# HengyiWang/spann3r

Measured on AMD Instinct MI355X. Metric: frames/sec/GPU (224px, 10-frame seq) + mem-bank cross-attn HBM GB/s, higher is better.
Workload: dtype bf16; 1 GPU; Spann3R.forward, 10-frame 224x224 sequence, batch 1, ViT-L enc / ViT-B dec / DPT heads, eval memory policy; parallelism=sequences sharded 1/GPU x1, hip_graphs=True

## Files before the change

include/spann3r_hip.h:

```cpp
#ifndef SPANN3R_HIP_H
#define SPANN3R_HIP_H

#include <stdint.h>

#ifdef __cplusplus
extern "C" {
#endif

enum { SP3_F32 = 0, SP3_BF16 = 1 };
enum { SP3_ATTN_F32X3 = 2, SP3_ATTN_F16X3 = 3 };
enum { SP3_ACT_NONE = 0, SP3_ACT_GELU = 1, SP3_ACT_RELU = 2 };
enum { SP3_EPI_PLAIN = 0, SP3_EPI_ROPE_VT = 1, SP3_EPI_PIXSHUF = 2, SP3_EPI_PARTIAL = 3 };
enum { SP3_LOAD_PLAIN = 0, SP3_LOAD_CONV3X3 = 1, SP3_LOAD_SOFTMAX = 2 };

const char* sp3_last_error(void);
int sp3_version(void);

int sp3_weight_stream_set(int mode);
int sp3_weight_stream_get(void);

typedef struct sp3_gemm_desc {
  const float* A;
  const float* A2;
  const void* W;
// ... 151 lines not shown
int sp3_gather_cols(const void* src, int64_t ld_src, void* dst, int64_t ld_dst, const int32_t* sel, int n_sel,
                    int n_fill, int C, int elem_size, void* stream);
int sp3_gather_1d(const float* src, float* dst, const int32_t* sel, int n_sel, void* stream);

int sp3_conv3x3_tile(const void* x, int in_bf16, const void* w_packed, const float* bias, const float* res1,
                     const float* res2, void* out, int out_bf16, int res_bf16, int tile_px, int B, int H, int W,
                     int Cin, int Cout, int relu_in, int act, void* stream);
int sp3_im2col_patch(const float* img, int64_t sb, int64_t sc, int64_t sy, int64_t sx, int B, int C, int H, int W,
                     int p, void* out, int out_bf16, int out_packed, void* stream);
int sp3_upsample2x(const float* in, float* out, int B, int H, int W, int C, int outH, int outW, void* stream);
int sp3_upsample2x_bf16(const void* in, void* out, int B, int H, int W, int C, int outH, int outW, void* stream);
int sp3_head_final(const float* feat, const float* w, const float* b, int64_t pixels, int C, float* pts,
                   float* conf, float* raw, void* stream);
int sp3_head_final_bf16(const void* feat, const float* w, const float* b, int64_t pixels, int C, float* pts, float* conf,
                        float* raw, void* stream);

int sp3_preprocess_image(const uint8_t* src, int64_t src_row_stride, int crop_l, int crop_t, int H1, int W1,
                         const int32_t* hbounds, const int32_t* hcoef, int hksize, int W2,
                         const int32_t* vbounds, const int32_t* vcoef, int vksize, int H2,
                         int crop2_l, int crop2_t, int outW, int outH, int transpose, uint8_t* tmp, float* out, void* stream);

int64_t sp3_conf_loss_ws_bytes(int n, int B);
int sp3_conf_loss_forward(const float* P, const float* Cf, const float* G, const uint8_t* V, const float* pose0, int n, int B, int HW,
                          float alpha, int fix_first, void* ws, float* out7, float* ent_out, void* stream);
int sp3_conf_loss_backward(const float* P, const float* Cf, const float* G, const uint8_t* V, const float* pose0, int n, int B, int HW,
                           float alpha, int fix_first, const void* ws, const float* grad_scale2, float* dP, float* dC, void* stream);
int64_t sp3_ssi_loss_ws_bytes(int n, int B, int HW);
int sp3_ssi_loss_forward(const float* P, const float* G, const uint8_t* V, const float* pose0, int n, int B, int HW, int fix_first,
                         int gt_scale, void* ws, float* out, void* stream);
int sp3_ssi_align_stats(const float* P, const float* G, const uint8_t* V, const float* pose0, int n, int B, int HW, void* ws, float* stats,
// ... 353 lines not shown
```

spann3r_amd/csrc/common.h:

```cpp
#pragma once
#include <hip/hip_runtime.h>
#include <stdint.h>
#include <stdio.h>
#include "../../include/spann3r_hip.h"

typedef __attribute__((ext_vector_type(8))) __bf16 bf16x8;
typedef __attribute__((ext_vector_type(4))) __bf16 bf16x4;
typedef __attribute__((ext_vector_type(2))) __bf16 bf16x2;
typedef __attribute__((ext_vector_type(4))) float f32x4;

#define SP3_WAVE 64

void sp3_set_error(const char* fmt, ...);

#define SP3_CHECK(cond, ...)                     \
  do {                                           \
    if (!(cond)) {                               \
      sp3_set_error(__VA_ARGS__);                \
      return 1;                                  \
    }                                            \
  } while (0)

#define SP3_LAUNCH_CHECK(what)                                              \
  do {                                                                      \
// ... 107 lines not shown
  return t;
}
__device__ __forceinline__ float up2x_mix(const Up2xTaps& t, float v00, float v01, float v10, float v11) {
  const float top = __fmaf_rn(t.hx, v00, __fmul_rn(t.lx, v01)), bot = __fmaf_rn(t.hx, v10, __fmul_rn(t.lx, v11));
  return __fmaf_rn(t.hy, top, __fmul_rn(t.ly, bot));
}

__device__ __forceinline__ int64_t packed_off(int row, int k, int K, bool bf16) {
  const int lkb = bf16 ? 6 : 5, lch = bf16 ? 4 : 3;
  const int nkb = (K + (1 << lkb) - 1) >> lkb;
  const int kb = k >> lkb, kk = k & ((1 << lkb) - 1);
  const int g = kk >> lch, e = kk & ((1 << lch) - 1);
  const int h = e >> (lch - 1), eh = e & ((1 << (lch - 1)) - 1);
  return (((((int64_t)(row >> 4) * nkb + kb) * 2 + h) * 4 + g) * 16 + (row & 15)) * (1 << (lch - 1)) + eh;
}
```

spann3r_amd/csrc/conv.hip:

```cpp
#include "common.h"
#include <type_traits>
#include <cstdlib>

namespace {

constexpr int TH = 8, TW = 8;
constexpr int HP = (TH + 2) * (TW + 2);
constexpr int BM = TH * TW, BN = 64;
constexpr int MF = BM / 16, NF = BN / 16;
constexpr int SLAB_LD = BN + 4;
constexpr int DEPTH = 3;
constexpr int SP3_CONV_WIDE_MIN_WGS = 256;

struct ConvArgs {
  const void* x; const __bf16* w; const float* bias; const float* res1; const float* res2; void* out;
  int B, H, W, Cin, Cout, tiles_x, tiles_y, relu_in, act, out_bf16;
  int xcd_nb;
};

__device__ __forceinline__ bool conv_tile_of(const ConvArgs& a, int& t, int& nblk) {
  t = blockIdx.x; nblk = blockIdx.y;
  if (a.xcd_nb) {
    const unsigned L = blockIdx.x, xc = L & 7, jj = L >> 3, q = jj / (unsigned)a.xcd_nb;
    nblk = (int)(jj - q * a.xcd_nb);
// ... 371 lines not shown

template <typename TIN, int NF, bool WS>
int launch(dim3 grid, hipStream_t st, const ConvArgs& a) {
  constexpr int lds = lds_bytes<NF>();
  auto kern = conv3x3_wide_kernel<TIN, NF, 0, WS>;
  if (lds > 64 * 1024) {
    static bool raised = false;
    if (!raised) {
      hipError_t e = hipFuncSetAttribute(reinterpret_cast<const void*>(kern), hipFuncAttributeMaxDynamicSharedMemorySize, lds);
      if (e != hipSuccess) { sp3_set_error("sp3_conv3x3_tile: cannot raise dynamic LDS to %d: %s", lds, hipGetErrorString(e)); return 2; }
      raised = true;
    }
  }
  hipLaunchKernelGGL(kern, grid, dim3(256), lds, st, a);
  return 0;
}
}

}

extern "C" int sp3_conv3x3_tile(const void* x, int in_bf16, const void* w_packed, const float* bias, const float* res1,
                                const float* res2, void* out, int out_bf16, int res_bf16, int tile_px, int B, int H, int W,
                                int Cin, int Cout, int relu_in, int act, void* stream) {
  SP3_CHECK(x && w_packed && out, "sp3_conv3x3_tile: null pointer");
  SP3_CHECK(B > 0 && H > 0 && W > 0, "sp3_conv3x3_tile: bad shape");
  SP3_CHECK(Cin % 64 == 0 && Cin >= 64 && Cout % 64 == 0 && Cout >= 64, "sp3_conv3x3_tile: Cin=%d / Cout=%d must be multiples of 64", Cin, Cout);
  SP3_CHECK(act == SP3_ACT_NONE || act == SP3_ACT_RELU, "sp3_conv3x3_tile: act %d", act);
  SP3_CHECK(out_bf16 == 0 || out_bf16 == 1, "sp3_conv3x3_tile: out_bf16 %d is not 0 or 1", out_bf16);
  SP3_CHECK(res_bf16 == 0 || res_bf16 == 1, "sp3_conv3x3_tile: res_bf16 %d is not 0 or 1", res_bf16);
  SP3_CHECK(tile_px >= 0 && tile_px <= 3, "sp3_conv3x3_tile: tile_px %d is not 0..3", tile_px);
// ... 38 lines not shown
  auto launch = [&](auto kern) -> int {
    static size_t raised = 0;
    if (lds > 64 * 1024 && lds > raised) {
      raised = lds;
      hipError_t e = hipFuncSetAttribute(reinterpret_cast<const void*>(kern), hipFuncAttributeMaxDynamicSharedMemorySize, (int)lds);
      if (e != hipSuccess) { sp3_set_error("sp3_conv3x3_tile: cannot raise dynamic LDS to %zu: %s", lds, hipGetErrorString(e)); return 2; }
    }
    hipLaunchKernelGGL(kern, grid, dim3(256), lds, st, a);
    return 0;
  };
  const int rc = in_bf16 ? launch(conv3x3_tile_kernel<__bf16>) : launch(conv3x3_tile_kernel<float>);
  if (rc) return rc;
  SP3_LAUNCH_CHECK("sp3_conv3x3_tile");
  return 0;
}
```

spann3r_amd/csrc/dpt.hip:

```cpp
#include "common.h"
#include <math.h>

namespace {

__global__ __launch_bounds__(256) void im2col_patch_kernel(const float* __restrict__ img, int64_t sb, int64_t sc, int64_t sy,
                                                           int64_t sx, int C, int H, int W, int p, void* __restrict__ out,
                                                           int out_bf16, int out_packed, int64_t total) {
  const int64_t idx = (int64_t)blockIdx.x * 256 + threadIdx.x;
  if (idx >= total) return;
  const int K = C * p * p;
  const int64_t row = idx / K;
  const int k = (int)(idx - row * K);
  const int nw = W / p, nh = H / p;
  const int b = (int)(row / (nh * nw));
  const int rem = (int)(row - (int64_t)b * nh * nw);
  const int ty = rem / nw, tx = rem - ty * nw;
  const int c = k / (p * p), r2 = k - c * p * p;
  const int iy = r2 / p, ix = r2 - iy * p;
  const float val = img[b * sb + c * sc + (int64_t)(ty * p + iy) * sy + (int64_t)(tx * p + ix) * sx];
  const int64_t o = out_packed ? packed_off((int)row, k, K, out_bf16 != 0) : idx;
  if (out_bf16) reinterpret_cast<__bf16*>(out)[o] = (__bf16)val;
  else reinterpret_cast<float*>(out)[o] = val;
}

// ... 91 lines not shown
    const float4 w1 = *reinterpret_cast<const float4*>(w + C + c);
    const float4 w2 = *reinterpret_cast<const float4*>(w + 2 * C + c);
    const float4 w3 = *reinterpret_cast<const float4*>(w + 3 * C + c);
    a0 += (x.x * w0.x + x.y * w0.y) + (x.z * w0.z + x.w * w0.w);
    a1 += (x.x * w1.x + x.y * w1.y) + (x.z * w1.z + x.w * w1.w);
    a2 += (x.x * w2.x + x.y * w2.y) + (x.z * w2.z + x.w * w2.w);
    a3 += (x.x * w3.x + x.y * w3.y) + (x.z * w3.z + x.w * w3.w);
  }
#pragma unroll
  for (int o = 1; o < 8; o <<= 1) {
    a0 += __shfl_xor(a0, o); a1 += __shfl_xor(a1, o); a2 += __shfl_xor(a2, o); a3 += __shfl_xor(a3, o);
  }
  if (valid && sub == 0) {
    const float x = a0 + bias[0], y = a1 + bias[1], z = a2 + bias[2], c = a3 + bias[3];
    if (raw) { raw[pix * 4 + 0] = x; raw[pix * 4 + 1] = y; raw[pix * 4 + 2] = z; raw[pix * 4 + 3] = c; }
    const float d = sqrtf(x * x + y * y + z * z);
    const float sc = expm1f(d) / fmaxf(d, 1e-8f);
    pts[pix * 3 + 0] = x * sc; pts[pix * 3 + 1] = y * sc; pts[pix * 3 + 2] = z * sc;
    conf[pix] = 1.0f + expf(c);
  }
}

template <int LP, int PPT>
__global__ __launch_bounds__(256) void head_final_bf16x8_kernel(const __bf16* __restrict__ feat, const float* __restrict__ w,
                                                                const float* __restrict__ bias, int64_t pixels, float* __restrict__ pts,
                                                                float* __restrict__ conf, float* __restrict__ raw) {
  constexpr int C = 8 * LP, PPB = 256 / LP;
  const int li = threadIdx.x % LP, pl = threadIdx.x / LP;
  float wr[4][8];
#pragma unroll
  for (int f = 0; f < 4; ++f) {
    const float4 a = *reinterpret_cast<const float4*>(w + f * C + li * 8), b = *reinterpret_cast<const float4*>(w + f * C + li * 8 + 4);
    wr[f][0] = a.x; wr[f][1] = a.y; wr[f][2] = a.z; wr[f][3] = a.w; wr[f][4] = b.x; wr[f][5] = b.y; wr[f][6] = b.z; wr[f][7] = b.w;
  }
// ... 12 lines not shown
    float a[4];
#pragma unroll
    for (int f = 0; f < 4; ++f) {
      float t0 = 0.f, t1 = 0.f;
#pragma unroll
      for (int e = 0; e < 4; ++e) { t0 = fmaf((float)x[q][e], wr[f][e], t0); t1 = fmaf((float)x[q][4 + e], wr[f][4 + e], t1); }
      a[f] = t0 + t1;
    }
#pragma unroll
    for (int o = 1; o < LP; o <<= 1) {
      a[0] += __shfl_xor(a[0], o); a[1] += __shfl_xor(a[1], o); a[2] += __shfl_xor(a[2], o); a[3] += __shfl_xor(a[3], o);
    }
    if (li == 0 && pix < pixels) {
      const float X = a[0] + b0, Y = a[1] + b1, Z = a[2] + b2, Cc = a[3] + b3;
      if (raw) *reinterpret_cast<float4*>(raw + pix * 4) = make_float4(X, Y, Z, Cc);
      const float d = sqrtf(X * X + Y * Y + Z * Z);
      const float sc = expm1f(d) / fmaxf(d, 1e-8f);
      pts[pix * 3 + 0] = X * sc; pts[pix * 3 + 1] = Y * sc; pts[pix * 3 + 2] = Z * sc;
      conf[pix] = 1.0f + expf(Cc);
    }
  }
}

}

#define ST(s) reinterpret_cast<hipStream_t>(s)

extern "C" int sp3_im2col_patch(const float* img, int64_t sb, int64_t sc, int64_t sy, int64_t sx, int B, int C, int H, int W,
                                int p, void* out, int out_bf16, int out_packed, void* stream) {
  SP3_CHECK(img && out && B > 0 && C > 0 && p > 0, "sp3_im2col_patch: bad arguments");
  SP3_CHECK(H % p == 0 && W % p == 0, "Input image size (%d,%d) is not a multiple of patch size (%d)", H, W, p);
  const int64_t total = (int64_t)B * (H / p) * (W / p) * C * p * p;
  hipLaunchKernelGGL(im2col_patch_kernel, dim3((unsigned)((total + 255) / 256)), dim3(256), 0, ST(stream), img, sb, sc, sy, sx,
                     C, H, W, p, out, out_bf16, out_packed, total);
// ... 57 lines not shown
```

spann3r_amd/engine.py:

```python
import math
import os

import torch

from . import ops
from .lib import ACT_NONE, ACT_GELU, ACT_RELU
from .config import Spann3RConfig


def _rope_tables(max_pos, base, device):
    half = 32
    inv_freq = 1.0 / (base ** (torch.arange(0, half, 2).float() / half))
    t = torch.arange(max_pos, dtype=torch.float32)
    ang = torch.einsum("i,j->ij", t, inv_freq)
    return ang.cos().contiguous().to(device), ang.sin().contiguous().to(device)


def _rope_tables_narrow(max_pos, base, head_dim, device):
    D = head_dim // 2
    nf = D // 2
    assert nf <= 16 and head_dim % 4 == 0
    inv_freq = 1.0 / (base ** (torch.arange(0, D, 2).float() / D))
    t = torch.arange(max_pos, dtype=torch.float32)
    ang = torch.einsum("i,j->ij", t, inv_freq)
# ... 576 lines not shown
        if x1 is not None:
            s = self.ws("fus_sum_" + tag, (M, F), self.mdt)
            self._rcu(x1, pre + "u1", B, H, W_, s, extra_res=x0, tag=tag, c1_done=c1_done, extra_up=x0_up)
            cur = s
        r = self.ws("fus_rcu2_" + tag, (M, F), self.mdt)
        self._rcu(cur, pre + "u2", B, H, W_, r, tag=tag, c1_done=c1_done and x1 is None)
        oc = self.ws("fus_oc_" + tag, (M, F), self.mdt)
        ops.gemm(r, w[pre + "out.w"], oc, M=M, N=F, K=F, lda=F, ldc=F, bias=w[pre + "out.b"])
        OH, OW = (2 * H, 2 * W_) if crop is None else crop
        if fold_up:
            return oc, OH, OW
        up = self.ws("fus_up_" + tag, (B * OH * OW, F), self.mdt)
        ops.upsample2x(oc, up, B=B, H=H, W_=W_, C_=F, outH=OH, outW=OW)
        return up, OH, OW

    def dpt_head(self, dec, B, nh, nw, num, want_raw=False):
        self.activate()
        cfg, w = self.cfg, self.w
        F, Lc = cfg.dpt_feat, cfg.dpt_last
        pre = "dpt%d." % num
        R = B * nh * nw
        hk = cfg.hooks
        dims = (cfg.enc_dim, cfg.dec_dim, cfg.dec_dim, cfg.dec_dim)
        ld = (96, 192, 384, 768)
        mdt = self.mdt
        t = [self.ws("dpt%d_pp%d" % (num, i), (R, ld[i]), mdt) for i in range(4)]
        import contextlib
        lv = ops.HEAD_LEVELS
        group = ops.level if len({dec[hk[i]].dtype for i in range(4)}) == 1 else contextlib.nullcontext
        with (group if lv else contextlib.nullcontext)():
            for i0 in (0, 2):
# ... 39 lines not shown
            for i in range(4):
                layer_rn(i)
        path, up, Hc, Wc = rn[3], None, h3, w3
        for j in range(4):
            Hn, Wn = geo[3 - j]
            fold = lv and j < 3 and ops.conv3x3_takes_res2_up(w[refs[j + 1][0] + "u1c2.w"], mdt, B, *geo[2 - j])
            nxt, OH_, OW_ = self._fusion(refs[j][0], B, Hn, Wn, path, rn[3 - j] if j else None, refs[j][1], crop=(nh, nw) if j == 0 else None,
                                         c1_done=lv, x0_up=up, fold_up=fold)
            path, up = nxt, ((Hn, Wn) if fold else None)
        p1, H1, W1 = path, OH_, OW_
        a = self.ws("dpt%d_h0" % num, (B * H1 * W1, Lc), mdt)
        ops.conv3x3(p1, w[pre + "h0.w"], a, B=B, H=H1, W_=W1, Cin=F, Cout=Lc, bias=w[pre + "h0.b"])
        OH, OW = 2 * H1, 2 * W1
        u = self.ws("dpt%d_h0up" % num, (B * OH * OW, Lc), mdt)
        ops.upsample2x(a, u, B=B, H=H1, W_=W1, C_=Lc)
        c = self.ws("dpt%d_h2" % num, (B * OH * OW, Lc), mdt)
        ops.conv3x3(u, w[pre + "h2.w"], c, B=B, H=OH, W_=OW, Cin=Lc, Cout=Lc, bias=w[pre + "h2.b"], act=ACT_RELU)
        pts = self.ws("dpt_pts%d" % num, (B, OH, OW, 3))
        conf = self.ws("dpt_conf%d" % num, (B, OH, OW))
        raw = self.ws("dpt_raw%d" % num, (B, OH, OW, 4)) if want_raw else None
        ops.head_final(c, w[pre + "h4.w"], w[pre + "h4.b"], B * OH * OW, Lc, pts, conf, raw)
        return pts, conf, raw

    def encode_cur_value_feat(self, tok, out, res, pos32=None):
        self.activate()
        cfg, w = self.cfg, self.w
        B, P, Cv = tok.shape
        assert Cv == cfg.val_dim
        R, E = B * P, cfg.enc_dim
        zero_pos = self.ws("valf_zero_pos", (R, 2), torch.int32, zero=True)
        rope_tab = None
        if cfg.mem_pos_enc:
            assert pos32 is not None and self.rope_narrow is not None
            zero_pos, rope_tab = pos32, self.rope_narrow
        x = self.ws("valf_x", (R, Cv))
        xpA, xpB = self.wsp("valf_xpA", R, Cv), self.wsp("valf_xpB", R, Cv)
        stA, stB = self.stats("valf_stA", R, Cv), self.stats("valf_stB", R, Cv)
        ops.copy2d(tok.reshape(R, Cv), Cv, x, Cv, R, Cv)
        ops.pack_stats(x, xpA, stA, rows=R, C_=Cv)
        for i in range(cfg.val_depth):
            self._block(x, xpA, stA, xpB, stB, R, B, P, Cv, cfg.enc_heads, "val%d." % i, zero_pos, tag="_valf",
                        head_dim=Cv // cfg.enc_heads, rope_tab=rope_tab)
        ops.gemm(xpA, w["value_out.w"], out, M=R, N=E, K=Cv, lda=Cv, ldc=E, bias=w["value_out.b"], res1=res, ldr1=E,
                 ln=ops.LnFold(stA, Cv, w["value_out.s"], 1e-6))
        return out

    def encode_cur_value(self, pts3d, out, res):
        self.activate()
        cfg, w = self.cfg, self.w
        B, H, W_, _ = pts3d.shape
        p, E = cfg.patch, cfg.enc_dim
        nh, nw = H // p, W_ // p
        P = nh * nw
        R = B * P
        _, pos32, zero_pos = self.positions(B, nh, nw)
        col = self.wsp("im2col_val", R, 3 * p * p)
        sb, sy, sx, sc = pts3d.stride()
        ops.im2col_patch(pts3d, col, B=B, C_=3, H=H, W_=W_, p=p, strides=(sb, sc, sy, sx))
        x, xp, st = self._vit(col, R, B, P, "pospatch", "val", cfg.val_depth, pos32 if cfg.mem_pos_enc else zero_pos, tag="_val")
        ops.gemm(xp, w["value_out.w"], out, M=R, N=E, K=E, lda=E, ldc=E, bias=w["value_out.b"], res1=res, ldr1=E,
                 ln=ops.LnFold(st, E, w["value_out.s"], 1e-6))
        return out
```

spann3r_amd/lib.py:

```python
import ctypes as C
import os

import torch

_HERE = os.path.dirname(os.path.abspath(__file__))
LIB_PATH = os.environ.get("SP3_LIB_PATH") or os.path.join(_HERE, "libspann3r_hip.so")

F32, BF16 = 0, 1
ATTN_F32X3, ATTN_F16X3 = 2, 3
ACT_NONE, ACT_GELU, ACT_RELU = 0, 1, 2
EPI_PLAIN, EPI_ROPE_VT, EPI_PIXSHUF, EPI_PARTIAL = 0, 1, 2, 3
LOAD_PLAIN, LOAD_CONV3X3, LOAD_SOFTMAX = 0, 1, 2


class GemmDesc(C.Structure):
    _fields_ = [
        ("A", C.c_void_p), ("A2", C.c_void_p), ("W", C.c_void_p), ("C", C.c_void_p), ("bias", C.c_void_p),
        ("res1", C.c_void_p), ("res2", C.c_void_p),
        ("M", C.c_int32), ("N", C.c_int32), ("K", C.c_int32), ("batch", C.c_int32),
        ("K1", C.c_int32),
        ("lda", C.c_int64), ("lda2", C.c_int64), ("ldw", C.c_int64), ("ldc", C.c_int64),
        ("ldr1", C.c_int64), ("ldr2", C.c_int64),
        ("strideA", C.c_int64), ("strideW", C.c_int64), ("strideC", C.c_int64),
        ("alpha", C.c_float), ("wdtype", C.c_int32), ("act", C.c_int32), ("out_bf16", C.c_int32),
# ... 158 lines not shown
    "sp3_cos_sim": [C.c_void_p, C.c_void_p, C.c_int, C.c_int, C.c_int, C.c_void_p, C.c_void_p, C.c_void_p],
    "sp3_mem_append": [C.c_void_p, C.c_void_p, C.c_int, C.c_int, C.c_void_p],
    "sp3_bank_state_set": [C.c_void_p, C.c_int, C.c_int, C.c_void_p],
    "sp3_prob_merge": [C.c_void_p, C.c_void_p, C.c_int, C.c_int, C.c_int, C.c_void_p, C.c_void_p],
    "sp3_colsum_prob": [C.c_void_p, C.c_void_p, C.c_int, C.c_int, C.c_int, C.c_void_p, C.c_void_p, C.c_void_p],
    "sp3_cos_sim_state": [C.c_void_p, C.c_void_p, C.c_int, C.c_int, C.c_int, C.c_void_p, C.c_void_p, C.c_void_p, C.c_void_p],
    "sp3_prune_select": [C.c_void_p, C.c_void_p, C.c_int, C.c_float, C.c_int, C.c_void_p, C.c_void_p],
    "sp3_gather_rows": [C.c_void_p, C.c_void_p, C.c_void_p, C.c_int, C.c_int, C.c_int, C.c_void_p],
    "sp3_gather_cols": [C.c_void_p, C.c_int64, C.c_void_p, C.c_int64, C.c_void_p, C.c_int, C.c_int, C.c_int,
                        C.c_int, C.c_void_p],
    "sp3_gather_1d": [C.c_void_p, C.c_void_p, C.c_void_p, C.c_int, C.c_void_p],
    "sp3_im2col_patch": [C.c_void_p, C.c_int64, C.c_int64, C.c_int64, C.c_int64, C.c_int, C.c_int, C.c_int, C.c_int,
                         C.c_int, C.c_void_p, C.c_int, C.c_int, C.c_void_p],
    "sp3_conv3x3_tile": [C.c_void_p, C.c_int, C.c_void_p, C.c_void_p, C.c_void_p, C.c_void_p, C.c_void_p, C.c_int, C.c_int, C.c_int,
                         C.c_int, C.c_int, C.c_int, C.c_int, C.c_int, C.c_int, C.c_int, C.c_void_p],
    "sp3_upsample2x": [C.c_void_p, C.c_void_p, C.c_int, C.c_int, C.c_int, C.c_int, C.c_int, C.c_int, C.c_void_p],
    "sp3_head_final": [C.c_void_p, C.c_void_p, C.c_void_p, C.c_int64, C.c_int, C.c_void_p, C.c_void_p, C.c_void_p,
                       C.c_void_p],
    "sp3_upsample2x_bf16": [C.c_void_p, C.c_void_p, C.c_int, C.c_int, C.c_int, C.c_int, C.c_int, C.c_int, C.c_void_p],
    "sp3_head_final_bf16": [C.c_void_p, C.c_void_p, C.c_void_p, C.c_int64, C.c_int, C.c_void_p, C.c_void_p, C.c_void_p,
                            C.c_void_p],
    "sp3_fill_f32": [C.c_void_p, C.c_float, C.c_int64, C.c_void_p],
    "sp3_cast_f32_to_bf16": [C.c_void_p, C.c_void_p, C.c_int64, C.c_void_p],
    "sp3_copy2d_f32": [C.c_void_p, C.c_int64, C.c_void_p, C.c_int64, C.c_int, C.c_int, C.c_void_p],
    "sp3_spin": [C.c_int64, C.c_void_p, C.c_void_p],
    "sp3_conf_loss_forward": [C.c_void_p, C.c_void_p, C.c_void_p, C.c_void_p, C.c_void_p, C.c_int, C.c_int, C.c_int, C.c_float, C.c_int,
                              C.c_void_p, C.c_void_p, C.c_void_p, C.c_void_p],
    "sp3_conf_loss_backward": [C.c_void_p, C.c_void_p, C.c_void_p, C.c_void_p, C.c_void_p, C.c_int, C.c_int, C.c_int, C.c_float, C.c_int,
                               C.c_void_p, C.c_void_p, C.c_void_p, C.c_void_p, C.c_void_p],
    "sp3_transpose": [C.c_void_p, C.c_int64, C.c_void_p, C.c_int64, C.c_int, C.c_int, C.c_void_p],
# ... 231 lines not shown
```

spann3r_amd/model.py:

```python
import argparse
import collections
import os
import weakref

import torch
import torch.nn as nn

from . import ops
from .config import Spann3RConfig, FULL
from .engine import Engine
from .weights import param_spec, alias_of, synth_state_dict


def _build_param_tree(root: nn.Module, spec):
    made = {}
    for key, shape in spec.items():
        parts = key.split(".")
        mod = root
        for name in parts[:-1]:
            if not hasattr(mod, name) or not isinstance(getattr(mod, name), nn.Module):
                mod.add_module(name, nn.Module())
            mod = getattr(mod, name)
        src = alias_of(key)
        if src is not None:
# ... 701 lines not shown
        if has_next:
            main.wait_stream(st[3])
        self.dec = (dec1, dec2)
        self.dec2_hooks = [dec2[h] for h in self.model.cfg.hooks[1:]]

    def _part2(self):
        eng, mem, B = self.eng, self.mem, self.B
        dec1, dec2 = self.dec
        main = torch.cuda.current_stream()
        st = eng.side_streams()
        pts2 = conf2 = None
        if not self.defer2:
            st[2].wait_stream(main)
            with torch.cuda.stream(st[2]):
                pts2, conf2, _ = eng.dpt_head(dec2, B, self.hh, self.hw, 2)
        pts1, conf1, _ = eng.dpt_head(dec1, B, self.hh, self.hw, 1)
        if eng.cfg.use_feat:
            eng.encode_cur_value_feat(dec1[-1], self.v, self.k1,
                                      pos32=eng.positions(B, self.nh, self.nw)[1] if eng.cfg.mem_pos_enc else None)
        else:
            eng.encode_cur_value(pts1.swapaxes(1, 2) if self.swap else pts1, self.v, self.k1)
        mem.stage_write(self.k1, self.v)
        if not self.defer2:
            main.wait_stream(st[2])
        self.out = (pts1, conf1, pts2, conf2)

    def run(self, first, has_next, use_graphs, post_copies=(), stream=False):
        mem = self.mem
        has_next = has_next and not self.batched
        gk = mem.graph_key()
        per_length = 0 if gk[0] in ("s", "p") else 1 if (stream or mem.state is not None) else self._out_steps
        if not use_graphs and ops._prof is not None:
            ops._prof.step_begin()
        need_sim = not self.training and mem.sim_needed()
        if need_sim:
            mem.arm_score_poll()
# ... 473 lines not shown
```

spann3r_amd/ops.py:

```python
import ctypes as C

import torch

from . import lib as L
from .lib import GemmDesc, F32, BF16, ATTN_F32X3, ATTN_F16X3, ACT_NONE, ACT_GELU, ACT_RELU


_prof = None


class Profiler:

    def __init__(self, blocker_ms=12.0):
        self.rec = []
        self.regions = []
        self.blocker_cycles = int(blocker_ms * 2.4e6)

    def step_begin(self):
        torch.cuda._sleep(self.blocker_cycles)

    def region_begin(self):
        return (self.begin(), len(self.rec))

    def region_end(self, key, e0, nbytes, info=None):
# ... 64 lines not shown
               37: "lean-stream-k3072-48x32xk8", 38: "lean-stream-k1792-64x32xk7",
               39: "lean-stream-k1024-48x32xk8", 40: "lean-conv-16x16xk12", 41: "lean-conv-32x32xk8", 42: "lean-packed-splitA-k1792-64x32xk7", 43: "lean-score-k1024-32x32xk8", 44: "lean-softmax-pv-16x64xk8",
               45: "lean-prob-k1024-256x128", 46: "lean-prob-pv-256x128",
               50: "lean-rope-k1024-256x128", 51: "lean-rope-k1024-128x128", 52: "lean-rope-k768-128x128", 53: "lean-packed-k1024-256x128",
               54: "lean-packed-k1024-128x128", 55: "lean-packed-k768-128x128", 56: "lean-stream-k1024-128x64", 57: "lean-stream-k4096-128x64",
               58: "lean-stream-k768-128x64", 59: "lean-stream-k3072-128x64", 60: "lean-stream-k1792-128x64",
               61: "lean-stream-k1024-256x128", 62: "lean-stream-k4096-256x128", 63: "lean-rope-k768-256x128", 64: "lean-packed-k768-256x128", 65: "lean-rope-k768-128x64", 66: "lean-packed-splitA-k1792-128x128", 67: "lean-packed-splitA-k1792-256x128"}


import os as _os
import threading as _threading
PROF_SHAPES = _os.environ.get("SP3_PROF_SHAPES", "0")[:1] == "1"
LEAN = _os.environ.get("SP3_LEAN_GEMM", "1")[:1] != "0"

HEAD_LEVELS = _os.environ.get("SP3_HEAD_LEVELS", "1")[:1] != "0"
_held = None


def level_block_map(problems):
    start = [0]
    for tile, M, N in problems:
        bm = 16 if tile == 40 else 32
        start.append(start[-1] + 8 * ((M + bm - 1) // bm) * ((N // bm + 7) // 8))

    def f(w):
        p = max(i for i in range(len(problems)) if w >= start[i])
        tile, M, N = problems[p]
        bm = 16 if tile == 40 else 32
        mt = (M + bm - 1) // bm
        local = w - start[p]
# ... 377 lines not shown
    d.tile = tile
    if S > 1:
        d.C, d.bias, d.res1, d.res2 = splitk_ws.data_ptr(), None, None, None
        d.act, d.epi, d.tile, d.splitk = ACT_NONE, L.EPI_PARTIAL, 0, S
    global _held
    held, _held = _held, None
    try:
        _gemm_launch(d, "sp3_gemm(conv3x3)", "conv3x3")
    finally:
        _held = held
    if S > 1:
        reduce_ln(splitk_ws, S, M, Cout, bias=bias, res=res1, ldres=Cout, x_out=out, ldx=Cout, act=act, res2=res2, ldres2=Cout)
    return out


def conv3x3_takes_res2_up(Wp, map_dtype, B, H, W_):
    d = _conv_desc(Wp, map_dtype, map_dtype, map_dtype, B=B, H=H, W_=W_, Cin=Wp.K // 9, Cout=Wp.N, stride=1, act=ACT_NONE, relu_in=False,
                   res2_up=((H + 1) // 2, (W_ + 1) // 2))
    d.res1 = d.res2 = 4096
    return _conv_route(d, Wp) == "lean"


def conv_splitk(M, N, K, wdtype):
    tiles = ((M + 31) // 32) * ((N + 31) // 32)
    nkb = K // (64 if wdtype == torch.bfloat16 else 32)
    s = 1
    while tiles * s * 2 <= 512 and nkb // (s * 2) >= 4 and s < 8:
        s *= 2
    return s

# ... 343 lines not shown
```

Baseline: 658.5 frames/s.

## Fuse DPT head final conv3x3 with 1x1 head, postprocess and value-patch im2col

Adds a conv3x3_head kernel that computes the last 128-channel 3x3 conv of the DPT head and then, in the epilogue, applies ReLU, the 4-output 1x1 projection (reduced with DPP), the depth/confidence postprocess, and optionally writes the packed bf16 im2col patch rows for the value encoder. This removes the 128-channel intermediate map write and read, the separate head_final launch, and the im2col_patch launch in encode_cur_value. In exchange, one block processes both 64-channel output halves serially, which adds LDS staging and reduces parallelism within that conv.

```diff
diff --git a/include/spann3r_hip.h b/include/spann3r_hip.h
--- a/include/spann3r_hip.h
+++ b/include/spann3r_hip.h
@@ -189,6 +189,9 @@
                    float* conf, float* raw, void* stream);
 int sp3_head_final_bf16(const void* feat, const float* w, const float* b, int64_t pixels, int C, float* pts, float* conf,
                         float* raw, void* stream);
+int sp3_conv3x3_head(const void* x, const void* w_packed, const float* bias, const float* head_w, const float* head_b,
+                     float* pts, float* conf, float* raw, void* patch, int B, int H, int W, int Cin, int Cout, int relu_in,
+                     void* stream);
 
 int sp3_preprocess_image(const uint8_t* src, int64_t src_row_stride, int crop_l, int crop_t, int H1, int W1,
                          const int32_t* hbounds, const int32_t* hcoef, int hksize, int W2,
diff --git a/spann3r_amd/csrc/common.h b/spann3r_amd/csrc/common.h
--- a/spann3r_amd/csrc/common.h
+++ b/spann3r_amd/csrc/common.h
@@ -145,3 +145,9 @@
   const int h = e >> (lch - 1), eh = e & ((1 << (lch - 1)) - 1);
   return (((((int64_t)(row >> 4) * nkb + kb) * 2 + h) * 4 + g) * 16 + (row & 15)) * (1 << (lch - 1)) + eh;
 }
+
+__device__ __forceinline__ float4 head_postprocess(float X, float Y, float Z, float Cc) {
+  const float d = sqrtf(X * X + Y * Y + Z * Z);
+  const float sc = expm1f(d) / fmaxf(d, 1e-8f);
+  return make_float4(X * sc, Y * sc, Z * sc, 1.0f + expf(Cc));
+}
diff --git a/spann3r_amd/csrc/conv.hip b/spann3r_amd/csrc/conv.hip
--- a/spann3r_amd/csrc/conv.hip
+++ b/spann3r_amd/csrc/conv.hip
@@ -409,6 +409,202 @@
   }
   hipLaunchKernelGGL(kern, grid, dim3(256), lds, st, a);
   return 0;
+}
+struct HeadArgs {
+  const float* head_w; const float* head_b; float* pts; float* conf; float* raw; __bf16* patch;
+};
+template <int CTRL> __device__ __forceinline__ float dpp_row(float v) {
+  return __builtin_bit_cast(float, __builtin_amdgcn_update_dpp(0, __builtin_bit_cast(int, v), CTRL, 0xf, 0xf, false));
+}
+constexpr int DPP_XOR1 = 0xB1, DPP_XOR2 = 0x4E, DPP_HALF_MIRROR = 0x141, DPP_ROW_MIRROR = 0x140;
+constexpr int HEAD_PART_OFF = lds_bytes<4>();
+constexpr int HEAD_STAGE_OFF = HEAD_PART_OFF + TH * TW * 16;
+constexpr int HEAD_LDS_BYTES = HEAD_STAGE_OFF + 3 * TH * TW * 4;
+
+__global__ __launch_bounds__(256, 2) void conv3x3_head_kernel(const ConvArgs a, const HeadArgs hd) {
+  constexpr int NF = 4, SLAB_LD = 68, DEPTH = 3;
+  extern __shared__ __attribute__((aligned(16))) char lds[];
+  const int tid = threadIdx.x, lane = tid & 63, wave = tid >> 6, g = lane >> 4, r = lane & 15;
+  const int Cin = a.Cin;
+  int t = blockIdx.x;
+  const int tx = t % a.tiles_x; t /= a.tiles_x;
+  const int ty = t % a.tiles_y;
+  const int b = t / a.tiles_y;
+  const int y0 = ty * TH, x0 = tx * TW;
+  const int nchunk = Cin / CH, upt = Cin >> 5;
+  const int total = 9 * nchunk;
+
+  typedef __attribute__((ext_vector_type(4))) uint32_t u32x4;
+  const int nkb = (9 * Cin) >> 6;
+  const uint32_t panel_bytes = (uint32_t)nkb * 128 * 8 * 2;
+  const auto wrsrc = __builtin_amdgcn_make_buffer_rsrc(const_cast<char*>(reinterpret_cast<const char*>(a.w)), 0, (int)(2 * NF * panel_bytes), 0x00020000);
+  const uint32_t wlane = (uint32_t)lane * 16 + (uint32_t)(wave & 1) * 1024;
+  const int wave_u = __builtin_amdgcn_readfirstlane(wave);
+  auto w_off_seq = [&](int blk, int seq) -> uint32_t {
+    seq = seq < total ? seq : total - 1;
+    const int c = seq / 9;
+    return (uint32_t)blk * NF * panel_bytes + (uint32_t)(((seq - 9 * c) * upt + 4 * c + wave_u) >> 1) * 2048;
+  };
+  auto w_load = [&](uint32_t o, bf16x8* dst) {
+#pragma unroll
+    for (int n = 0; n < NF; ++n) {
+      const u32x4 v = __builtin_amdgcn_raw_buffer_load_b128(wrsrc, wlane, o + n * panel_bytes, SP3_AUX_DEFAULT);
+      dst[n] = *reinterpret_cast<const bf16x8*>(&v);
+    }
+  };
+
+  const char* abase = lds + r * PS + (((wave >> 1) << 6) + 16 * g + ((wave & 1) << 3)) * 2;
+  constexpr int CPP = CH / 8, PSTEP = 256 / CPP, NB = 12;
+  static_assert(NB * PSTEP >= HP, "one batch holds the halo chunk");
+  const uint32_t img_bytes = (uint32_t)(a.H * a.W * Cin) * 2u;
+  const auto rsrc = __builtin_amdgcn_make_buffer_rsrc(
+      const_cast<char*>(reinterpret_cast<const char*>(a.x)) + (int64_t)b * img_bytes, 0, (int)img_bytes, 0x00020000);
+
+  float4* part = reinterpret_cast<float4*>(lds + HEAD_PART_OFF);
+  float* stage = reinterpret_cast<float*>(lds + HEAD_STAGE_OFF);
+
+#pragma nounroll
+  for (int blk = 0; blk < 2; ++blk) {
+    bf16x8 wq[DEPTH][NF];
+#pragma unroll
+    for (int s = 0; s < DEPTH; ++s) w_load(w_off_seq(blk, s), wq[s]);
+    f32x4 acc[MF][NF];
+#pragma unroll
+    for (int m = 0; m < MF; ++m)
+#pragma unroll
+      for (int n = 0; n < NF; ++n) acc[m][n] = f32x4{0.f, 0.f, 0.f, 0.f};
+    int tidh = tid, y0h = y0, x0h = x0;
+    asm volatile("" : "+v"(tidh), "+s"(y0h), "+s"(x0h));
+    const uint32_t xlane = (uint32_t)((tidh % CPP) * 16);
+    char* hdst = lds + (tidh % CPP) * 16;
+    for (int c = 0; c < nchunk; ++c) {
+      if (blk | c) __syncthreads();
+      {
+        const int p0 = tidh / CPP;
+        u32x4 buf[NB];
+#pragma unroll
+        for (int q = 0; q < NB; ++q) {
+          const int p = p0 + q * PSTEP;
+          const int hy = p / HW, hx = p - hy * HW;
+          const int iy = y0h + hy - 1, ix = x0h + hx - 1;
+          const bool ok = p < HP && iy >= 0 && iy < a.H && ix >= 0 && ix < a.W;
+          const uint32_t off = ok ? (uint32_t)((iy * a.W + ix) * Cin + c * CH) * 2u + xlane : 0x80000000u;
+          buf[q] = __builtin_amdgcn_raw_buffer_load_b128(rsrc, off, 0, 0);
+        }
+#pragma unroll
+        for (int q = 0; q < NB; ++q) {
+          const int p = p0 + q * PSTEP;
+          if (p >= HP) continue;
+          u32x4 v = buf[q];
+          if (a.relu_in) {
+#pragma unroll
+            for (int e = 0; e < 4; ++e) {
+              const uint32_t neg = v[e] & 0x80008000u;
+              v[e] &= ~((neg >> 15) * 0xffffu);
+            }
+          }
+          *reinterpret_cast<u32x4*>(hdst + p * PS) = v;
+        }
+      }
+      __syncthreads();
+
+      bf16x8 af[MF];
+#pragma unroll
+      for (int m = 0; m < MF; ++m) af[m] = ld_frag_lds(abase + m * HW * PS);
+#pragma unroll
+      for (int tap = 0; tap < 9; ++tap) {
+        const int s = tap % DEPTH;
+        const int nt = tap + 1, nky = nt / 3, nkx = nt - 3 * nky;
+#pragma unroll
+        for (int m = 0; m < MF; ++m) {
+#pragma unroll
+          for (int n = 0; n < NF; ++n)
+            acc[m][n] = __builtin_amdgcn_mfma_f32_16x16x32_bf16(af[m], wq[s][n], acc[m][n], 0, 0, 0);
+          if (tap < 8) af[m] = ld_frag_lds(abase + ((m + nky) * HW + nkx) * PS);
+        }
+        w_load(w_off_seq(blk, 9 * c + tap + DEPTH), wq[s]);
+      }
+    }
+
+    int tide = tid, y0e = y0, x0e = x0;
+    asm volatile("" : "+v"(tide), "+s"(y0e), "+s"(x0e));
+    const int j = tide & 15, c4 = 4 * j, rx = tide >> 4;
+    float* slab = reinterpret_cast<float*>(lds) + (size_t)wave * 64 * SLAB_LD;
+    const float* sm = reinterpret_cast<const float*>(lds) + c4;
+    const int n0 = 64 * blk;
+    const float4 cb = *reinterpret_cast<const float4*>(a.bias + n0 + c4);
+    float4 hw[4];
+#pragma unroll
+    for (int f = 0; f < 4; ++f) hw[f] = *reinterpret_cast<const float4*>(hd.head_w + f * 128 + n0 + c4);
+#pragma unroll
+    for (int h = 0; h < 2; ++h) {
+      __syncthreads();
+#pragma unroll
+      for (int m = 0; m < 4; ++m)
+#pragma unroll
+        for (int n = 0; n < NF; ++n)
+#pragma unroll
+          for (int q = 0; q < 4; ++q) slab[(m * 16 + 4 * g + q) * SLAB_LD + n * 16 + r] = acc[4 * h + m][n][q];
+      __syncthreads();
+#pragma unroll
+      for (int it = 0; it < 4; ++it) {
+        const int row = it * 16 + rx, ry = 4 * h + it;
+        float4 v = *reinterpret_cast<const float4*>(sm + row * SLAB_LD);
+#pragma unroll
+        for (int s = 1; s < 4; ++s) {
+          const float4 t4 = *reinterpret_cast<const float4*>(sm + (size_t)s * 64 * SLAB_LD + row * SLAB_LD);
+          v.x += t4.x; v.y += t4.y; v.z += t4.z; v.w += t4.w;
+        }
+        v.x += cb.x; v.y += cb.y; v.z += cb.z; v.w += cb.w;
+        v = relu4(v);
+        const float x0f = (float)(__bf16)v.x, x1f = (float)(__bf16)v.y, x2f = (float)(__bf16)v.z, x3f = (float)(__bf16)v.w;
+        float o[4];
+#pragma unroll
+        for (int f = 0; f < 4; ++f) {
+          float tt = 0.f;
+          tt = fmaf(x0f, hw[f].x, tt); tt = fmaf(x1f, hw[f].y, tt); tt = fmaf(x2f, hw[f].z, tt); tt = fmaf(x3f, hw[f].w, tt);
+          tt = tt + dpp_row<DPP_XOR1>(tt);
+          tt += dpp_row<DPP_XOR2>(tt);
+          tt += dpp_row<DPP_HALF_MIRROR>(tt);
+          o[f] = tt + dpp_row<DPP_ROW_MIRROR>(tt);
+        }
+        if (j == 0) {
+          if (blk == 0) {
+            part[ry * TW + rx] = make_float4(o[0], o[1], o[2], o[3]);
+          } else {
+            const int oy = y0e + ry, ox = x0e + rx;
+            if (oy < a.H && ox < a.W) {
+              const float4 s0 = part[ry * TW + rx];
+              const float X = (s0.x + o[0]) + hd.head_b[0], Y = (s0.y + o[1]) + hd.head_b[1], Z = (s0.z + o[2]) + hd.head_b[2],
+                          Cc = (s0.w + o[3]) + hd.head_b[3];
+              const int64_t pix = ((int64_t)b * a.H + oy) * a.W + ox;
+              if (hd.raw) *reinterpret_cast<float4*>(hd.raw + pix * 4) = make_float4(X, Y, Z, Cc);
+              const float4 pc = head_postprocess(X, Y, Z, Cc);
+              hd.pts[pix * 3 + 0] = pc.x; hd.pts[pix * 3 + 1] = pc.y; hd.pts[pix * 3 + 2] = pc.z;
+              hd.conf[pix] = pc.w;
+              if (hd.patch) {
+                stage[0 * TH * TW + ry * TW + rx] = pc.x; stage[1 * TH * TW + ry * TW + rx] = pc.y; stage[2 * TH * TW + ry * TW + rx] = pc.z;
+              }
+            }
+          }
+        }
+      }
+    }
+  }
+  if (hd.patch) {
+    __syncthreads();
+    if (tid < 3 * TH * 2) {
+      const int c = tid >> 4, ry = (tid >> 1) & 7, hx = tid & 1;
+      const float* src = stage + c * TH * TW + ry * TW + 8 * hx;
+      bf16x8 o;
+#pragma unroll
+      for (int e = 0; e < 8; ++e) o[e] = (__bf16)src[e];
+      const int nw = a.W >> 4, nh = a.H >> 4;
+      const int prow = (b * nh + (y0 >> 4)) * nw + (x0 >> 4);
+      const int k = c * 256 + ((y0 & 15) + ry) * 16 + 8 * hx;
+      *reinterpret_cast<bf16x8*>(hd.patch + packed_off(prow, k, 768, true)) = o;
+    }
+  }
 }
 }
 
@@ -477,3 +673,34 @@
   SP3_LAUNCH_CHECK("sp3_conv3x3_tile");
   return 0;
 }
+
+extern "C" int sp3_conv3x3_head(const void* x, const void* w_packed, const float* bias, const float* head_w, const float* head_b,
+                                float* pts, float* conf, float* raw, void* patch, int B, int H, int W, int Cin, int Cout,
+                                int relu_in, void* stream) {
+  SP3_CHECK(x && w_packed && bias && head_w && head_b && pts && conf, "sp3_conv3x3_head: null pointer");
+  SP3_CHECK(B > 0 && H > 0 && W > 0, "sp3_conv3x3_head: bad shape");
+  SP3_CHECK(Cin == wide::CH && Cout == 128, "sp3_conv3x3_head: Cin=%d / Cout=%d must both be 128", Cin, Cout);
+  SP3_CHECK(!patch || (H % 16 == 0 && W % 16 == 0), "sp3_conv3x3_head: patch rows need H %% 16 == 0 and W %% 16 == 0 (H=%d, W=%d)", H, W);
+  auto al16 = [](const void* q) { return (reinterpret_cast<uintptr_t>(q) & 15) == 0; };
+  SP3_CHECK(al16(x) && al16(w_packed) && al16(bias) && al16(head_w) && al16(raw) && al16(patch), "sp3_conv3x3_head: 16-byte alignment");
+  SP3_CHECK((int64_t)H * W * Cin * 2 < (1ll << 31), "sp3_conv3x3_head: one image of the map must stay below 2 GiB");
+  ConvArgs a;
+  a.x = x; a.w = reinterpret_cast<const __bf16*>(w_packed); a.bias = bias; a.res1 = nullptr; a.res2 = nullptr; a.out = nullptr;
+  a.B = B; a.H = H; a.W = W; a.Cin = Cin; a.Cout = Cout;
+  a.relu_in = relu_in; a.act = SP3_ACT_RELU; a.out_bf16 = 1; a.xcd_nb = 1;
+  a.tiles_x = (W + wide::TW - 1) / wide::TW; a.tiles_y = (H + wide::TH - 1) / wide::TH;
+  const int64_t tiles = (int64_t)a.tiles_x * a.tiles_y * B;
+  SP3_CHECK(tiles < (1ll << 31), "sp3_conv3x3_head: %lld pixel tiles", (long long)tiles);
+  wide::HeadArgs hd;
+  hd.head_w = head_w; hd.head_b = head_b; hd.pts = pts; hd.conf = conf; hd.raw = raw; hd.patch = reinterpret_cast<__bf16*>(patch);
+  static bool raised = false;
+  if (!raised) {
+    hipError_t e = hipFuncSetAttribute(reinterpret_cast<const void*>(wide::conv3x3_head_kernel), hipFuncAttributeMaxDynamicSharedMemorySize,
+                                       wide::HEAD_LDS_BYTES);
+    if (e != hipSuccess) { sp3_set_error("sp3_conv3x3_head: cannot raise dynamic LDS to %d: %s", wide::HEAD_LDS_BYTES, hipGetErrorString(e)); return 2; }
+    raised = true;
+  }
+  hipLaunchKernelGGL(wide::conv3x3_head_kernel, dim3((unsigned)tiles), dim3(256), wide::HEAD_LDS_BYTES, reinterpret_cast<hipStream_t>(stream), a, hd);
+  SP3_LAUNCH_CHECK("sp3_conv3x3_head");
+  return 0;
+}
diff --git a/spann3r_amd/csrc/dpt.hip b/spann3r_amd/csrc/dpt.hip
--- a/spann3r_amd/csrc/dpt.hip
+++ b/spann3r_amd/csrc/dpt.hip
@@ -129,10 +129,9 @@
   if (valid && sub == 0) {
     const float x = a0 + bias[0], y = a1 + bias[1], z = a2 + bias[2], c = a3 + bias[3];
     if (raw) { raw[pix * 4 + 0] = x; raw[pix * 4 + 1] = y; raw[pix * 4 + 2] = z; raw[pix * 4 + 3] = c; }
-    const float d = sqrtf(x * x + y * y + z * z);
-    const float sc = expm1f(d) / fmaxf(d, 1e-8f);
-    pts[pix * 3 + 0] = x * sc; pts[pix * 3 + 1] = y * sc; pts[pix * 3 + 2] = z * sc;
-    conf[pix] = 1.0f + expf(c);
+    const float4 pc = head_postprocess(x, y, z, c);
+    pts[pix * 3 + 0] = pc.x; pts[pix * 3 + 1] = pc.y; pts[pix * 3 + 2] = pc.z;
+    conf[pix] = pc.w;
   }
 }
 
@@ -175,10 +174,9 @@
     if (li == 0 && pix < pixels) {
       const float X = a[0] + b0, Y = a[1] + b1, Z = a[2] + b2, Cc = a[3] + b3;
       if (raw) *reinterpret_cast<float4*>(raw + pix * 4) = make_float4(X, Y, Z, Cc);
-      const float d = sqrtf(X * X + Y * Y + Z * Z);
-      const float sc = expm1f(d) / fmaxf(d, 1e-8f);
-      pts[pix * 3 + 0] = X * sc; pts[pix * 3 + 1] = Y * sc; pts[pix * 3 + 2] = Z * sc;
-      conf[pix] = 1.0f + expf(Cc);
+      const float4 pc = head_postprocess(X, Y, Z, Cc);
+      pts[pix * 3 + 0] = pc.x; pts[pix * 3 + 1] = pc.y; pts[pix * 3 + 2] = pc.z;
+      conf[pix] = pc.w;
     }
   }
 }
diff --git a/spann3r_amd/engine.py b/spann3r_amd/engine.py
--- a/spann3r_amd/engine.py
+++ b/spann3r_amd/engine.py
@@ -614,7 +614,14 @@
         ops.upsample2x(oc, up, B=B, H=H, W_=W_, C_=F, outH=OH, outW=OW)
         return up, OH, OW
 
-    def dpt_head(self, dec, B, nh, nw, num, want_raw=False):
+    def value_patch_buffer(self, B, nh, nw):
+        cfg = self.cfg
+        if (ops.HEAD_TAIL_FUSED and not cfg.use_feat and cfg.patch == 16 and self.adt == torch.bfloat16
+                and ops.head_tail_fused_ok(self.mdt, cfg.dpt_last, cfg.dpt_last, 16 * nh, 16 * nw, False)):
+            return self.wsp("im2col_val", B * nh * nw, 3 * 256)
+        return None
+
+    def dpt_head(self, dec, B, nh, nw, num, want_raw=False, patch_out=None):
         self.activate()
         cfg, w = self.cfg, self.w
         F, Lc = cfg.dpt_feat, cfg.dpt_last
@@ -684,11 +691,16 @@
         OH, OW = 2 * H1, 2 * W1
         u = self.ws("dpt%d_h0up" % num, (B * OH * OW, Lc), mdt)
         ops.upsample2x(a, u, B=B, H=H1, W_=W1, C_=Lc)
-        c = self.ws("dpt%d_h2" % num, (B * OH * OW, Lc), mdt)
-        ops.conv3x3(u, w[pre + "h2.w"], c, B=B, H=OH, W_=OW, Cin=Lc, Cout=Lc, bias=w[pre + "h2.b"], act=ACT_RELU)
         pts = self.ws("dpt_pts%d" % num, (B, OH, OW, 3))
         conf = self.ws("dpt_conf%d" % num, (B, OH, OW))
         raw = self.ws("dpt_raw%d" % num, (B, OH, OW, 4)) if want_raw else None
+        if ops.HEAD_TAIL_FUSED and ops.head_tail_fused_ok(mdt, Lc, Lc, OH, OW, want_raw):
+            ops.conv3x3_head(u, w[pre + "h2.w"], w[pre + "h2.b"], w[pre + "h4.w"], w[pre + "h4.b"], pts, conf, raw, patch_out,
+                             B=B, H=OH, W_=OW, Cin=Lc, Cout=Lc)
+            return pts, conf, raw
+        assert patch_out is None, "dpt_head: patch_out needs the fused head tail (value_patch_buffer)"
+        c = self.ws("dpt%d_h2" % num, (B * OH * OW, Lc), mdt)
+        ops.conv3x3(u, w[pre + "h2.w"], c, B=B, H=OH, W_=OW, Cin=Lc, Cout=Lc, bias=w[pre + "h2.b"], act=ACT_RELU)
         ops.head_final(c, w[pre + "h4.w"], w[pre + "h4.b"], B * OH * OW, Lc, pts, conf, raw)
         return pts, conf, raw
 
@@ -715,7 +727,7 @@
                  ln=ops.LnFold(stA, Cv, w["value_out.s"], 1e-6))
         return out
 
-    def encode_cur_value(self, pts3d, out, res):
+    def encode_cur_value(self, pts3d, out, res, col_done=False):
         self.activate()
         cfg, w = self.cfg, self.w
         B, H, W_, _ = pts3d.shape
@@ -726,7 +738,8 @@
         _, pos32, zero_pos = self.positions(B, nh, nw)
         col = self.wsp("im2col_val", R, 3 * p * p)
         sb, sy, sx, sc = pts3d.stride()
-        ops.im2col_patch(pts3d, col, B=B, C_=3, H=H, W_=W_, p=p, strides=(sb, sc, sy, sx))
+        if not col_done:
+            ops.im2col_patch(pts3d, col, B=B, C_=3, H=H, W_=W_, p=p, strides=(sb, sc, sy, sx))
         x, xp, st = self._vit(col, R, B, P, "pospatch", "val", cfg.val_depth, pos32 if cfg.mem_pos_enc else zero_pos, tag="_val")
         ops.gemm(xp, w["value_out.w"], out, M=R, N=E, K=E, lda=E, ldc=E, bias=w["value_out.b"], res1=res, ldr1=E,
                  ln=ops.LnFold(st, E, w["value_out.s"], 1e-6))
diff --git a/spann3r_amd/lib.py b/spann3r_amd/lib.py
--- a/spann3r_amd/lib.py
+++ b/spann3r_amd/lib.py
@@ -196,6 +196,8 @@
                          C.c_int, C.c_void_p, C.c_int, C.c_int, C.c_void_p],
     "sp3_conv3x3_tile": [C.c_void_p, C.c_int, C.c_void_p, C.c_void_p, C.c_void_p, C.c_void_p, C.c_void_p, C.c_int, C.c_int, C.c_int,
                          C.c_int, C.c_int, C.c_int, C.c_int, C.c_int, C.c_int, C.c_int, C.c_void_p],
+    "sp3_conv3x3_head": [C.c_void_p, C.c_void_p, C.c_void_p, C.c_void_p, C.c_void_p, C.c_void_p, C.c_void_p, C.c_void_p, C.c_void_p,
+                         C.c_int, C.c_int, C.c_int, C.c_int, C.c_int, C.c_int, C.c_void_p],
     "sp3_upsample2x": [C.c_void_p, C.c_void_p, C.c_int, C.c_int, C.c_int, C.c_int, C.c_int, C.c_int, C.c_void_p],
     "sp3_head_final": [C.c_void_p, C.c_void_p, C.c_void_p, C.c_int64, C.c_int, C.c_void_p, C.c_void_p, C.c_void_p,
                        C.c_void_p],
diff --git a/spann3r_amd/model.py b/spann3r_amd/model.py
--- a/spann3r_amd/model.py
+++ b/spann3r_amd/model.py
@@ -739,12 +739,13 @@
             st[2].wait_stream(main)
             with torch.cuda.stream(st[2]):
                 pts2, conf2, _ = eng.dpt_head(dec2, B, self.hh, self.hw, 2)
-        pts1, conf1, _ = eng.dpt_head(dec1, B, self.hh, self.hw, 1)
+        col = None if self.swap else eng.value_patch_buffer(B, self.hh, self.hw)
+        pts1, conf1, _ = eng.dpt_head(dec1, B, self.hh, self.hw, 1, patch_out=col)
         if eng.cfg.use_feat:
             eng.encode_cur_value_feat(dec1[-1], self.v, self.k1,
                                       pos32=eng.positions(B, self.nh, self.nw)[1] if eng.cfg.mem_pos_enc else None)
         else:
-            eng.encode_cur_value(pts1.swapaxes(1, 2) if self.swap else pts1, self.v, self.k1)
+            eng.encode_cur_value(pts1.swapaxes(1, 2) if self.swap else pts1, self.v, self.k1, col_done=col is not None)
         mem.stage_write(self.k1, self.v)
         if not self.defer2:
             main.wait_stream(st[2])
diff --git a/spann3r_amd/ops.py b/spann3r_amd/ops.py
--- a/spann3r_amd/ops.py
+++ b/spann3r_amd/ops.py
@@ -102,6 +102,7 @@
 LEAN = _os.environ.get("SP3_LEAN_GEMM", "1")[:1] != "0"
 
 HEAD_LEVELS = _os.environ.get("SP3_HEAD_LEVELS", "1")[:1] != "0"
+HEAD_TAIL_FUSED = _os.environ.get("SP3_HEAD_TAIL_FUSED", "1")[:1] != "0"
 _held = None
 
 
@@ -509,6 +510,30 @@
     return out
 
 
+def head_tail_fused_ok(map_dtype, Cin, Cout, H, W_, want_raw):
+    del want_raw
+    return (map_dtype == torch.bfloat16 and Cin == 128 and Cout == 128 and H > 0 and W_ > 0
+            and ((W_ + 15) // 16) * ((H + 7) // 8) >= 40)
+
+
+def conv3x3_head(x, Wp, bias, head_w, head_b, pts, conf, raw=None, patch=None, *, B, H, W_, Cin, Cout, relu_in=False):
+    if x.dtype != torch.bfloat16 or not x.is_cuda:
+        raise TypeError("conv3x3_head: the map must be a bfloat16 CUDA(HIP) tensor")
+    if not isinstance(Wp, PackedWeight) or Wp.dtype != torch.bfloat16:
+        raise TypeError("conv3x3_head: the weight must be a bf16 PackedWeight")
+    for t, n in ((bias, "bias"), (head_w, "head_w"), (head_b, "head_b"), (pts, "pts"), (conf, "conf"), (raw, "raw")):
+        _f32(t, n)
+    if patch is not None and not (isinstance(patch, PackedAct) and patch.dtype == torch.bfloat16 and patch.K == 768
+                                  and patch.M >= B * (H // 16) * (W_ // 16)):
+        raise TypeError("conv3x3_head: patch must be a bf16 PackedAct [>= B*(H/16)*(W/16), 768]")
+    px = B * H * W_
+    _timed("conv3x3_head", 2.0 * px * Cout * 9 * Cin + 8.0 * px * 128,
+           px * 2.0 * Cin + 2.0 * 9 * Cin * Cout + px * (16.0 + (1.5 if patch is not None else 0.0)),
+           lambda: L.check(L.load().sp3_conv3x3_head(
+               x.data_ptr(), Wp.data_ptr(), bias.data_ptr(), head_w.data_ptr(), head_b.data_ptr(), pts.data_ptr(), conf.data_ptr(),
+               L.ptr(raw), L.ptr(patch), B, H, W_, Cin, Cout, int(relu_in), L.stream_ptr()), "sp3_conv3x3_head"))
+
+
 def conv3x3_takes_res2_up(Wp, map_dtype, B, H, W_):
     d = _conv_desc(Wp, map_dtype, map_dtype, map_dtype, B=B, H=H, W_=W_, Cin=Wp.K // 9, Cout=Wp.N, stride=1, act=ACT_NONE, relu_in=False,
                    res2_up=((H + 1) // 2, (W_ + 1) // 2))
```

Result: no change. 661.7 frames/s (median of 6 runs) (+0.5%).
